# serviceberry3/weiner_slamit_v2

Measured on AMD Instinct MI355X. Metric: frames/sec ORB extract+match @640x480x8lvl, higher is better.
Workload: dtype u8; 1 GPU; BASELINE configs[1]: 640x480 8-level ORB extract (1000 features, FAST 20/7) + brute-force 256-bit Hamming best/second match vs the stream's previous frame; 256 independent streams per GPU per step; distinct_frame_pairs_per_gpu=16, parallelism=streams sharded over 1 GPU(s), no data-path collective

## Files before the change

weiner_slamit_v2_amd/csrc/orb_api.hip:

```cpp
#include <hip/hip_runtime.h>
#include <math.h>
#include <stdio.h>
#include <stdlib.h>
#include <string.h>

#include <algorithm>
#include <vector>

#include "../../include/slamit.h"
#include "orb_plan.h"
#include "slamit_internal.h"

hipError_t orbk_upload_pattern(hipStream_t st);
void orbk_resize(hipStream_t st, const uint8_t* src, int sw, int sh, size_t sstride, size_t sframe,
                 uint8_t* dst, int dw, int dh, size_t dstride, size_t dframe, const int* xofs,
                 const short* ialpha, const int* yofs, const short* ibeta, int nframes);
void orbk_resize_rows4(hipStream_t st, const uint8_t* src, size_t sstride, size_t sframe, int sh, uint8_t* dst, int dw, int dh,
                       size_t dstride, size_t dframe, const uint32_t* d_col, const uint32_t* d_row, int nframes);
void orbk_resize_rows8(hipStream_t st, const uint8_t* src, size_t sstride, size_t sframe, int sh, uint8_t* dst, int dw, int dh,
                       size_t dstride, size_t dframe, const uint32_t* d_col8, const uint32_t* d_row, int nframes);
hipError_t orbk_pyramid_prepare(int smem_bytes);
void orbk_pyramid(hipStream_t st, const OrbLevel* levels, int nlevels, const PyrBox* boxes, const PyrTabs* tabs,
                  int nregions, const uint8_t* img0, size_t img0_stride, size_t img0_frame, uint8_t* pyr, int bufA_bytes,
                  int smem_bytes, int nframes, int l_first, int l_last);
hipError_t orbk_fast_prepare(int max_wcell, int max_hcell);
void orbk_fast(hipStream_t st, const FastTab& tab, int nlevels, const uint32_t* d_cells, int cells_per_frame, const uint8_t* img0,
               size_t img0_stride, size_t img0_frame, const uint8_t* pyr, unsigned long long* cand,
               size_t cand_frame_stride, int* cand_count, int iniTh, int minTh, int max_wcell, int max_hcell, int nframes);
hipError_t orbk_octree_prepare(int node_cap, int key_cap);
void orbk_octree(hipStream_t st, const OrbLevel* levels, int nlevels, const unsigned long long* cand,
                 size_t cand_frame_stride, int* cand_count, uint32_t* ws_xy, uint16_t* ws_node,
                 OrbLevelKp* lkp, size_t kp_frame_stride, int* kp_count, int node_cap, int key_cap, int nframes,
                 int level_override);
void orbk_ic_angle(hipStream_t st, const OrbLevel* levels, int nlevels, const uint8_t* img0, size_t img0_stride,
                   size_t img0_frame, const uint8_t* pyr, OrbLevelKp* lkp, size_t kp_frame_stride,
                   const int* kp_count, int max_kp, int nframes);
void orbk_blur_stream(hipStream_t st, const OrbLevel* levels, const uint32_t* d_tiles, int ntiles, const uint8_t* img0,
                      size_t img0_stride, size_t img0_frame, const uint8_t* pyr, uint8_t* blur, int nframes, bool edge);
void orbk_blur(hipStream_t st, const OrbLevel* levels, const uint32_t* d_tiles, int total_tiles, const uint8_t* img0,
               size_t img0_stride, size_t img0_frame, const uint8_t* pyr, uint8_t* blur, int nframes);
void orbk_describe(hipStream_t st, const OrbLevel* levels, int nlevels, const uint8_t* blur,
                   const OrbLevelKp* lkp, size_t kp_frame_stride, const int* kp_count, slamit_kp* out_kps,
                   uint8_t* out_desc, int out_cap, int* out_n, int max_kp, int nframes);
void orbk_pad(hipStream_t st, const uint8_t* src, int w, int h, size_t sstride, uint8_t* dst);
void orbk_decode_candidates(hipStream_t st, const OrbLevel* levels, int level, const unsigned long long* K, int n,
                            unsigned long long* order_out, int* xys);

namespace {

inline size_t round_up(size_t v, size_t a) { return (v + a - 1) / a * a; }

}

#define ORB_BLUR_SPLIT 1

struct slamit_orb {
    slamit_orb_params p;
    int device;
    hipStream_t stream;
    hipStream_t stream_b;
    hipEvent_t ev_pyr, ev_mid, ev_blur;
    SlamitSwitches sw;
    int nlevels;
    OrbPlan pl;
    bool blur_stream_on;
    uint8_t* d_tables;
    const OrbLevel* d_levels;
    uint8_t* d_pyr;
    uint8_t* d_blur;
    unsigned long long* d_cand;
    uint32_t* d_ws_xy;
    uint16_t* d_ws_node;
    int* d_counts;
// ... 43 lines not shown
        p->ini_th_fast < 1 || p->ini_th_fast > 255 || p->min_th_fast < 1 || p->min_th_fast > 255 ||
        p->width < 0 || p->height < 0 || p->max_batch < 1)
        return slamit_fail(SLAMIT_ERR_ARG, "slamit_orb_create: parameter out of range");
    SLAMIT_USE_DEVICE(device);
    slamit_orb* h = new slamit_orb();
    h->p = *p;
    h->device = device;
    h->sw = slamit_read_switches();
    const int nl = h->nlevels = p->nlevels;
    const char* why = "";
    if (!orb_plan(*p, OrbPlanOptions{h->sw.resize_no8}, h->pl, &why)) {
        delete h;
        return slamit_fail(SLAMIT_ERR_ARG, why);
    }
    const OrbPlan& P = h->pl;
    const bool empty = P.levels.empty();
    h->blur_stream_on = !empty && !h->sw.blur_no_stream;

    const size_t B = (size_t)p->max_batch;
    const size_t counts_bytes = sizeof(int) * ((ORB_CC_PAD + 1) * B * nl + 2 * ORB_CC_PAD);
    h->d_in_stride = round_up((size_t)std::max(p->width, 1), 64);
    h->d_in_frame = h->d_in_stride * std::max(p->height, 1);
    h->scratch_bytes = std::max<size_t>((size_t)(p->width + 38) * (p->height + 38),
                                        (sizeof(unsigned long long) + 3 * sizeof(int)) * (P.cand_frame_stride + 64));
    hipError_t e = hipSuccess;
#define ALLOC(ptr, bytes) if (e == hipSuccess) e = hipMalloc((void**)&(ptr), std::max<size_t>((bytes), 256))
    ALLOC(h->d_tables, P.table_bytes);
    ALLOC(h->d_pyr, P.pyr_frame_total * B);
    ALLOC(h->d_blur, P.blur_frame_total * B + 256);
    ALLOC(h->d_cand, sizeof(unsigned long long) * P.cand_frame_stride * B);
    ALLOC(h->d_ws_xy, sizeof(uint32_t) * P.cand_frame_stride * B);
    ALLOC(h->d_ws_node, sizeof(uint16_t) * P.cand_frame_stride * B);
    ALLOC(h->d_counts, counts_bytes);
    ALLOC(h->d_lkp, sizeof(OrbLevelKp) * P.kp_frame_stride * B);
    ALLOC(h->d_in, h->d_in_frame * B);
    ALLOC(h->d_out_kps, sizeof(slamit_kp) * (size_t)P.max_out * B);
    ALLOC(h->d_out_desc, (size_t)SLAMIT_DESC_BYTES * P.max_out * B);
    ALLOC(h->d_out_n, sizeof(int) * B);
    ALLOC(h->d_scratch, h->scratch_bytes);
#undef ALLOC
    if (e == hipSuccess) e = hipHostMalloc((void**)&h->h_out, 256 + (size_t)B * 256 + (sizeof(slamit_kp) + SLAMIT_DESC_BYTES) * (size_t)P.max_out * B, hipHostMallocDefault);
    if (e == hipSuccess) e = hipStreamCreateWithFlags(&h->stream, hipStreamNonBlocking);
    if (e == hipSuccess) e = hipStreamCreateWithFlags(&h->stream_b, hipStreamNonBlocking);
    if (e == hipSuccess) e = hipEventCreateWithFlags(&h->ev_pyr, hipEventDisableTiming);
    if (e == hipSuccess) e = hipEventCreateWithFlags(&h->ev_mid, hipEventDisableTiming);
    if (e == hipSuccess) e = hipEventCreateWithFlags(&h->ev_blur, hipEventDisableTiming);
    if (e == hipSuccess && P.table_bytes) {
        std::vector<uint8_t> img;
        orb_plan_image(P, h->d_tables, img);
        e = hipMemcpy(h->d_tables, img.data(), img.size(), hipMemcpyHostToDevice);
    }
    h->d_levels = dtab<OrbLevel>(h, P.levels_off);
    if (e == hipSuccess && P.pyr_regions) e = orbk_pyramid_prepare(P.pyr_smem);
    if (e == hipSuccess) e = orbk_upload_pattern(h->stream);
    if (e == hipSuccess) e = orbk_octree_prepare(P.node_cap, P.oct_key_cap);
    if (e == hipSuccess && !empty) e = orbk_fast_prepare(P.max_wcell, P.max_hcell);
    if (e == hipSuccess) e = hipMemset(h->d_counts, 0, counts_bytes);
    if (e == hipSuccess) e = hipStreamSynchronize(h->stream);
    if (e != hipSuccess) {
        orb_free(h);
        return slamit_fail_hip(e, "slamit_orb_create");
    }
    *out = h;
    return SLAMIT_OK;
}
void slamit_orb_destroy(slamit_orb* h) { orb_free(h); }

int slamit_orb_tables(const slamit_orb* h, float* scale, float* inv_scale, float* sigma2, float* inv_sigma2,
                      int32_t* features_per_level) {
    if (!h) return slamit_fail(SLAMIT_ERR_ARG, "slamit_orb_tables: null handle");
    for (int i = 0; i < h->nlevels; ++i) {
        if (scale) scale[i] = h->pl.scale[i];
        if (inv_scale) inv_scale[i] = h->pl.inv_scale[i];
        if (sigma2) sigma2[i] = h->pl.sigma2[i];
        if (inv_sigma2) inv_sigma2[i] = h->pl.inv_sigma2[i];
        if (features_per_level) features_per_level[i] = h->pl.per_level[i];
    }
    return SLAMIT_OK;
}

int slamit_orb_max_keypoints(const slamit_orb* h) { return h ? h->pl.max_out : 0; }

enum { ST_RESIZE = 0, ST_FAST, ST_OCTREE, ST_ANGLE, ST_BLUR, ST_DESCRIBE, ST_COUNT };

static void prof_mark(slamit_orb* h, hipStream_t st, int stage, bool begin) {
    if (!h->prof_on || h->prof_ev.size() >= 2 * 16384) return;
    if (h->prof_on >= 2 && (stage != ST_FAST || h->prof_call % (h->prof_on - 1) != 0)) return;
    hipEvent_t e;
    if (hipEventCreate(&e) != hipSuccess) return;
    hipEventRecord(e, st);
    h->prof_ev.push_back(e);
    if (begin) h->prof_stage.push_back(stage);
}

int slamit_orb_extract_batch_dev(slamit_orb* h, const uint8_t* d_gray, size_t stride, size_t frame_stride,
                                 int nframes, slamit_kp* d_kps, uint8_t* d_desc, int cap, int32_t* d_n_out,
                                 void* stream) {
    if (!h || !d_n_out || nframes < 0) return slamit_fail(SLAMIT_ERR_ARG, "slamit_orb_extract_batch_dev: bad argument");
    if (nframes > h->p.max_batch) return slamit_fail(SLAMIT_ERR_CAPACITY, "slamit_orb_extract_batch_dev: nframes > max_batch");
    if (nframes == 0) return SLAMIT_OK;
    SLAMIT_USE_DEVICE(h->device);
    hipStream_t st = stream ? (hipStream_t)stream : h->stream;
    const int nl = h->nlevels;
    const OrbPlan& P = h->pl;
    if (h->p.width == 0 || h->p.height == 0) {
        HIP_TRY(hipMemsetAsync(d_n_out, 0, sizeof(int) * nframes, st));
        h->last_nframes = 0;
        return SLAMIT_OK;
    }
    if (!d_gray || !d_kps || !d_desc) return slamit_fail(SLAMIT_ERR_ARG, "slamit_orb_extract_batch_dev: null buffer");
    if (cap < P.max_out) return slamit_fail(SLAMIT_ERR_CAPACITY, "slamit_orb_extract_batch_dev: cap < slamit_orb_max_keypoints()");
    if (stride < (size_t)h->p.width || (nframes > 1 && frame_stride < stride * (size_t)h->p.height))
        return slamit_fail(SLAMIT_ERR_ARG, "slamit_orb_extract_batch_dev: stride smaller than the frame");
    if (stride >= ((size_t)1 << 24)) return slamit_fail(SLAMIT_ERR_ARG, "slamit_orb_extract_batch_dev: row pitch of 16 MiB or more");
    int* cand_count = h->d_counts;
    int* kp_count = h->d_counts + (size_t)h->p.max_batch * nl * ORB_CC_PAD;
    if (!h->counters_clean) HIP_TRY(hipMemsetAsync(h->d_counts, 0, sizeof(int) * (size_t)h->p.max_batch * nl * ORB_CC_PAD, st));
    h->counters_clean = false;
    const bool blur_src_aligned = ((((uintptr_t)d_gray) | stride | frame_stride) & 3) == 0;
    auto launch_blur = [&](hipStream_t bs, int l0, int l1) {
        auto strips = [&](const OrbStrips& S) { return dtab<uint32_t>(h, S.off) + 4 * (size_t)S.base[l0]; };
        auto nstrips = [&](const OrbStrips& S) { return S.base[l1] - S.base[l0]; };
        if (h->blur_stream_on && blur_src_aligned) {
            orbk_blur_stream(bs, h->d_levels, strips(P.blur_str), nstrips(P.blur_str), d_gray, stride, frame_stride, h->d_pyr, h->d_blur, nframes, false);
            orbk_blur_stream(bs, h->d_levels, strips(P.blur_edge), nstrips(P.blur_edge), d_gray, stride, frame_stride, h->d_pyr, h->d_blur, nframes, true);
        } else {
            orbk_blur(bs, h->d_levels, strips(P.blur_all), nstrips(P.blur_all), d_gray, stride, frame_stride, h->d_pyr, h->d_blur, nframes);
        }
    };
    prof_mark(h, st, ST_RESIZE, true);
    const bool src0_aligned = ((((uintptr_t)d_gray) | stride | frame_stride) & 3) == 0;
    const bool side = h->prof_on != 1;
    const bool early_blur = side && ORB_BLUR_SPLIT < nl - 1;
    bool early_done = false;
    if (P.rows4_ok && src0_aligned) {
        for (int l = 1; l < nl; ++l) {
            const OrbLevel& S = P.levels[l - 1];
            const OrbLevel& D = P.levels[l];
            const uint8_t* src = l == 1 ? d_gray : h->d_pyr + S.plane_off;
            const OrbResizeTabs& T = P.rs[l];
            if (!T.col8.empty())
                orbk_resize_rows8(st, src, l == 1 ? stride : (size_t)S.stride, l == 1 ? frame_stride : P.pyr_frame_total, S.h,
                                  h->d_pyr + D.plane_off, D.w, D.h, (size_t)D.stride, P.pyr_frame_total, dtab<uint32_t>(h, T.col8_off),
                                  dtab<uint32_t>(h, T.row4_off), nframes);
            else
                orbk_resize_rows4(st, src, l == 1 ? stride : (size_t)S.stride, l == 1 ? frame_stride : P.pyr_frame_total, S.h,
                                  h->d_pyr + D.plane_off, D.w, D.h, (size_t)D.stride, P.pyr_frame_total, dtab<uint32_t>(h, T.col4_off),
                                  dtab<uint32_t>(h, T.row4_off), nframes);
            if (early_blur && l == ORB_BLUR_SPLIT) {
                HIP_TRY(hipEventRecord(h->ev_mid, st));
                HIP_TRY(hipStreamWaitEvent(h->stream_b, h->ev_mid, 0));
                launch_blur(h->stream_b, 0, l + 1);
                early_done = true;
            }
        }
    } else if (P.pyr_regions) {
        orbk_pyramid(st, h->d_levels, nl, dtab<PyrBox>(h, P.boxes_off), dtab<PyrTabs>(h, P.tabs_off), P.pyr_regions, d_gray, stride, frame_stride,
                     h->d_pyr, P.pyr_bufA, P.pyr_smem, nframes, 0, nl - 1);
    } else {
        for (int l = 1; l < nl; ++l) {
            const OrbLevel& S = P.levels[l - 1];
            const OrbLevel& D = P.levels[l];
            const uint8_t* src = l == 1 ? d_gray : h->d_pyr + S.plane_off;
            size_t sstride = l == 1 ? stride : (size_t)S.stride;
            size_t sframe = l == 1 ? frame_stride : P.pyr_frame_total;
            const OrbResizeTabs& T = P.rs[l];
            orbk_resize(st, src, S.w, S.h, sstride, sframe, h->d_pyr + D.plane_off, D.w, D.h, (size_t)D.stride,
                        P.pyr_frame_total, dtab<int>(h, T.xofs_off), dtab<short>(h, T.ialpha_off), dtab<int>(h, T.yofs_off),
                        dtab<short>(h, T.ibeta_off), nframes);
        }
    }
    prof_mark(h, st, ST_RESIZE, false);
    prof_mark(h, st, ST_FAST, true);
    orbk_fast(st, P.fast, nl, dtab<uint32_t>(h, P.cells_off), (int)(P.cells.size() / 4), d_gray, stride, frame_stride, h->d_pyr, h->d_cand,
              P.cand_frame_stride, cand_count, h->p.ini_th_fast, h->p.min_th_fast, P.max_wcell, P.max_hcell, nframes);
    prof_mark(h, st, ST_FAST, false);
    if (side) {
        HIP_TRY(hipEventRecord(h->ev_pyr, st));
        HIP_TRY(hipStreamWaitEvent(h->stream_b, h->ev_pyr, 0));
        launch_blur(h->stream_b, early_done ? ORB_BLUR_SPLIT + 1 : 0, nl);
        HIP_TRY(hipEventRecord(h->ev_blur, h->stream_b));
    }
    prof_mark(h, st, ST_OCTREE, true);
    orbk_octree(st, h->d_levels, nl, h->d_cand, P.cand_frame_stride, cand_count, h->d_ws_xy, h->d_ws_node, h->d_lkp,
                P.kp_frame_stride, kp_count, P.node_cap, P.oct_key_cap, nframes, -1);
    prof_mark(h, st, ST_OCTREE, false);
    prof_mark(h, st, ST_ANGLE, true);
    orbk_ic_angle(st, h->d_levels, nl, d_gray, stride, frame_stride, h->d_pyr, h->d_lkp, P.kp_frame_stride, kp_count,
                  P.max_kp_level, nframes);
    prof_mark(h, st, ST_ANGLE, false);
    if (side) {
        HIP_TRY(hipStreamWaitEvent(st, h->ev_blur, 0));
    } else {
        prof_mark(h, st, ST_BLUR, true);
        launch_blur(st, 0, nl);
        prof_mark(h, st, ST_BLUR, false);
    }
    prof_mark(h, st, ST_DESCRIBE, true);
    orbk_describe(st, h->d_levels, nl, h->d_blur, h->d_lkp, P.kp_frame_stride, kp_count, d_kps, d_desc, cap, d_n_out,
                  P.max_kp_level, nframes);
    prof_mark(h, st, ST_DESCRIBE, false);
    ++h->prof_call;
    HIP_TRY(hipGetLastError());
    h->counters_clean = true;
    h->last_img0 = d_gray; h->last_stride = stride; h->last_frame = frame_stride; h->last_nframes = nframes;
    return SLAMIT_OK;
}

int slamit_orb_extract_batch(slamit_orb* h, const uint8_t* gray, size_t stride, size_t frame_stride, int nframes,
                             slamit_kp* kps, uint8_t* desc, int cap, int* n_out) {
    if (!h || !n_out || nframes < 0) return slamit_fail(SLAMIT_ERR_ARG, "slamit_orb_extract_batch: bad argument");
    if (nframes > h->p.max_batch) return slamit_fail(SLAMIT_ERR_CAPACITY, "slamit_orb_extract_batch: nframes > max_batch");
    if (nframes == 0) return SLAMIT_OK;
    if (h->p.width == 0 || h->p.height == 0) {
        for (int f = 0; f < nframes; ++f) n_out[f] = 0;
        return SLAMIT_OK;
    }
    if (!gray || !kps || !desc) return slamit_fail(SLAMIT_ERR_ARG, "slamit_orb_extract_batch: null buffer");
    if (cap < h->pl.max_out) return slamit_fail(SLAMIT_ERR_CAPACITY, "slamit_orb_extract_batch: cap < slamit_orb_max_keypoints()");
    SLAMIT_USE_DEVICE(h->device);
    const int W = h->p.width, H = h->p.height;
    for (int f = 0; f < nframes; ++f)
        HIP_TRY(hipMemcpy2DAsync(h->d_in + f * h->d_in_frame, h->d_in_stride, gray + (size_t)f * frame_stride, stride, W, H,
                                 hipMemcpyHostToDevice, h->stream));
    int rc = slamit_orb_extract_batch_dev(h, h->d_in, h->d_in_stride, h->d_in_frame, nframes, h->d_out_kps, h->d_out_desc,
                                          h->pl.max_out, h->d_out_n, h->stream);
    if (rc != SLAMIT_OK) return rc;
    const size_t o_k = ((sizeof(int) * (size_t)nframes + 255) & ~(size_t)255), kb = sizeof(slamit_kp) * (size_t)h->pl.max_out * nframes;
    const size_t o_d = (o_k + kb + 255) & ~(size_t)255, db = (size_t)SLAMIT_DESC_BYTES * h->pl.max_out * nframes;
    HIP_TRY(hipMemcpyAsync(h->h_out, h->d_out_n, sizeof(int) * nframes, hipMemcpyDeviceToHost, h->stream));
    HIP_TRY(hipMemcpyAsync(h->h_out + o_k, h->d_out_kps, kb, hipMemcpyDeviceToHost, h->stream));
    HIP_TRY(hipMemcpyAsync(h->h_out + o_d, h->d_out_desc, db, hipMemcpyDeviceToHost, h->stream));
    HIP_TRY(hipStreamSynchronize(h->stream));
// ... 99 lines not shown
```

weiner_slamit_v2_amd/csrc/orb_kernels.hip:

```cpp
#include <hip/hip_runtime.h>
#include <stdint.h>

#include <algorithm>

#include "orb_types.h"
#include "slamit_math.h"
#include "../../include/slamit.h"
#include "../../include/slamit_orb_pattern.h"

#define WAVE 64

__global__ __launch_bounds__(256) void resize_level_kernel(
    const uint8_t* __restrict__ src, int sw, int sh, size_t sstride, size_t sframe,
    uint8_t* __restrict__ dst, int dw, int dh, size_t dstride, size_t dframe,
    const int* __restrict__ xofs, const short* __restrict__ ialpha,
    const int* __restrict__ yofs, const short* __restrict__ ibeta) {
    const int x4 = (blockIdx.x * 64 + (threadIdx.x & 63)) * 4;
    const int y = blockIdx.y * 4 + (threadIdx.x >> 6);
    const int f = blockIdx.z;
    if (x4 >= dw || y >= dh) return;
    const uint8_t* S = src + (size_t)f * sframe;
    int sy = yofs[y];
    int sy0 = min(max(sy, 0), sh - 1), sy1 = min(max(sy + 1, 0), sh - 1);
    const uint8_t* S0 = S + (size_t)sy0 * sstride;
// ... 120 lines not shown
        const unsigned srow = (r & 1) ? (rt[r >> 1].x >> 16) : (rt[r >> 1].x & 0xFFFFu);
        const unsigned ro = __umul24(srow, ss) + b;
        const rs_u4 v = __builtin_amdgcn_raw_buffer_load_b128(rsrc, (int)ro, 0, 0);
        w[r][0] = v.x; w[r][1] = v.y; w[r][2] = v.z; w[r][3] = v.w;
    }
#pragma unroll
    for (int k = 0; k < 2 * RP; ++k) {
        uint32_t h[2][8];
#pragma unroll
        for (int r = 0; r < 2; ++r) {
            const uint32_t* ww = w[2 * k + r];
            const uint32_t a0 = __builtin_amdgcn_alignbyte(ww[1], ww[0], sh), a1 = __builtin_amdgcn_alignbyte(ww[2], ww[1], sh), a2 = __builtin_amdgcn_alignbyte(ww[3], ww[2], sh);
#pragma unroll
            for (int j = 0; j < 4; ++j) h[r][j] = rs_dot2(__builtin_amdgcn_perm(a1, a0, sel[j]), al[j]) >> 4;
#pragma unroll
            for (int j = 4; j < 8; ++j) h[r][j] = rs_dot2(__builtin_amdgcn_perm(a2, a1, sel[j]), al[j]) >> 4;
        }
        const unsigned b0 = rt[k].y & 0xFFFFu, b1 = rt[k].y >> 16;
        uint32_t out[2] = {0, 0};
#pragma unroll
        for (int j = 0; j < 8; ++j) {
            const uint32_t v = ((__umul24(b0, h[0][j]) >> 16) + (__umul24(b1, h[1][j]) >> 16) + 2u) >> 2;
            out[j >> 2] |= (v & 0xFFu) << (8 * (j & 3));
        }
        *reinterpret_cast<uint2*>(D + (__umul24((unsigned)yrow[k], dstride) + 8u * (unsigned)g)) = make_uint2(out[0], out[1]);
    }
}

template <int RP>
__global__ __launch_bounds__(256) void resize_rows8_kernel(
    const uint8_t* __restrict__ src, size_t sstride, size_t sframe,
    uint8_t* __restrict__ dst, size_t dstride, size_t dframe,
    const uint4* __restrict__ coltab, const uint2* __restrict__ rowtab, int ngroups, unsigned inv_groups, int nitems, int dh, unsigned sbytes) {
    const int item = blockIdx.x * 256 + threadIdx.x;
    if (item >= nitems) return;
    rs_item8<RP>(item, src + (size_t)blockIdx.y * sframe, (unsigned)sstride, sbytes, dst + (size_t)blockIdx.y * dframe, (unsigned)dstride, coltab, rowtab,
                 ngroups, inv_groups, dh);
}

void orbk_resize_rows8(hipStream_t st, const uint8_t* src, size_t sstride, size_t sframe, int sh, uint8_t* dst, int dw, int dh,
                       size_t dstride, size_t dframe, const uint32_t* d_col8, const uint32_t* d_row, int nframes) {
    const int ng = (dw + 7) / 8, nitems = ng * ((dh + 2 * RS_RP - 1) / (2 * RS_RP));
    const unsigned inv = (unsigned)((0x100000000ull + (unsigned)ng - 1) / (unsigned)ng);
    hipLaunchKernelGGL(resize_rows8_kernel<RS_RP>, dim3((nitems + 255) / 256, nframes), dim3(256), 0, st, src, sstride, sframe, dst, dstride, dframe,
                       reinterpret_cast<const uint4*>(d_col8), reinterpret_cast<const uint2*>(d_row), ng, inv, nitems, dh, (unsigned)(sstride * (size_t)sh));
}

void orbk_resize_rows4(hipStream_t st, const uint8_t* src, size_t sstride, size_t sframe, int sh, uint8_t* dst, int dw, int dh,
                       size_t dstride, size_t dframe, const uint32_t* d_col, const uint32_t* d_row, int nframes) {
    const int ng = (dw + 3) / 4, nitems = ng * ((dh + 2 * RS_RP - 1) / (2 * RS_RP));
    const unsigned inv = (unsigned)((0x100000000ull + (unsigned)ng - 1) / (unsigned)ng);
    hipLaunchKernelGGL(resize_rows4_kernel<RS_RP>, dim3((nitems + 255) / 256, nframes), dim3(256), 0, st, src, sstride, sframe, dst, dstride, dframe,
                       reinterpret_cast<const uint4*>(d_col), reinterpret_cast<const uint2*>(d_row), ng, inv, nitems, dh, (unsigned)(sstride * (size_t)sh));
}

#define PYR_THREADS 512

__global__ __launch_bounds__(PYR_THREADS) void pyramid_fused_kernel(
    const OrbLevel* __restrict__ levels, int nlevels, const PyrBox* __restrict__ boxes,
    const PyrTabs* __restrict__ tabs, const uint8_t* __restrict__ img0, size_t img0_stride, size_t img0_frame,
    uint8_t* __restrict__ pyr, int bufA_bytes, int l_first, int l_last) {
    extern __shared__ __attribute__((aligned(16))) uint8_t pbuf[];
    uint8_t* buf[2] = {pbuf, pbuf + bufA_bytes};
    const int tx = threadIdx.x & 63, ty = threadIdx.x >> 6;
    const int PYR_ROWS = blockDim.x >> 6, NT = blockDim.x;
    const int frame = blockIdx.y;
    const PyrBox* B = boxes + (size_t)blockIdx.x * nlevels;
    {
        const PyrBox b = B[l_first];
        const int nw = b.nx1 - b.nx0, pitch = (nw + 3) & ~3;
        const uint8_t* S;
        size_t sstride;
        if (l_first == 0) { S = img0 + (size_t)frame * img0_frame; sstride = img0_stride; }
        else { S = pyr + levels[l_first].plane_off + (size_t)frame * levels[l_first].plane_bytes; sstride = (size_t)levels[l_first].stride; }
        const bool aligned = ((((uintptr_t)S) | sstride) & 3) == 0;
        const int w0 = levels[l_first].w;
        if (aligned) {
            const int nd = pitch >> 2;
            for (int y = b.ny0 + ty; y < b.ny1; y += PYR_ROWS)
                for (int d = tx; d < nd; d += 64) {
                    const int x = b.nx0 + 4 * d;
                    uint32_t v;
                    if (x + 4 <= w0) v = *reinterpret_cast<const uint32_t*>(S + (size_t)y * sstride + x);
                    else { v = 0; for (int j = 0; j < 4; ++j) if (x + j < w0) v |= (uint32_t)S[(size_t)y * sstride + x + j] << (8 * j); }
                    *reinterpret_cast<uint32_t*>(&buf[0][(y - b.ny0) * pitch + 4 * d]) = v;
                }
        } else {
            for (int y = b.ny0 + ty; y < b.ny1; y += PYR_ROWS)
                for (int x = b.nx0 + tx; x < b.nx1; x += 64)
                    buf[0][(y - b.ny0) * pitch + (x - b.nx0)] = S[(size_t)y * sstride + x];
        }
    }
    __syncthreads();
    for (int l = l_first + 1; l <= l_last; ++l) {
        const PyrBox b = B[l], pb = B[l - 1];
        const OrbLevel& L = levels[l];
        const int sw = levels[l - 1].w, sh = levels[l - 1].h;
        const PyrTabs T = tabs[l];
        const uint8_t* src = buf[(l - 1 - l_first) & 1];
        uint8_t* dst = buf[(l - l_first) & 1];
        const int spitch = ((pb.nx1 - pb.nx0) + 3) & ~3, dpitch = ((b.nx1 - b.nx0) + 3) & ~3;
        uint8_t* plane = pyr + L.plane_off + (size_t)frame * L.plane_bytes;
        const int nw = b.nx1 - b.nx0;
        int cx0[4], cx1[4], ca0[4], ca1[4];
        unsigned ownmask = 0;
#pragma unroll
// ... 1481 lines not shown
```

weiner_slamit_v2_amd/csrc/orb_plan.cc:

```cpp
#include "orb_plan.h"

#include <math.h>
#include <string.h>

#include <algorithm>

namespace {

inline int cv_round(double v) { return (int)lrint(v); }
inline size_t round_up(size_t v, size_t a) { return (v + a - 1) / a * a; }

inline short sat_short(float v) {
    int iv = cv_round((double)v);
    return (short)(iv < -32768 ? -32768 : iv > 32767 ? 32767 : iv);
}

void plan_scales(const slamit_orb_params& p, OrbPlan& P) {
    const int nl = p.nlevels;
    const double scaleFactor = (double)p.scale_factor;
    P.scale.assign(nl, 1.f); P.sigma2.assign(nl, 1.f); P.inv_scale.assign(nl, 1.f); P.inv_sigma2.assign(nl, 1.f);
    for (int i = 1; i < nl; ++i) {
        P.scale[i] = (float)(P.scale[i - 1] * scaleFactor);
        P.sigma2[i] = P.scale[i] * P.scale[i];
    }
// ... 205 lines not shown
            P.rows4_ok = false;
            T.col4.clear(); T.row4.clear();
        }
        if (o.resize_no8 || !rows8_table(D.w, S.w, (size_t)D.stride, T.xofs.data(), T.ialpha.data(), T.col8)) T.col8.clear();
    }
}

void plan_pyramid_boxes(const slamit_orb_params& p, OrbPlan& P) {
    const int nl = (int)P.levels.size(), last = nl - 1;
    if (nl < 2) return;
    const int GX = std::max(1, (p.width + 127) / 128), GY = std::max(1, (p.height + 95) / 96);
    std::vector<PyrBox> boxes((size_t)GX * GY * nl);
    bool ok = true;
    size_t capA = 16, capB = 16;
    for (int gy = 0; gy < GY && ok; ++gy)
        for (int gx = 0; gx < GX && ok; ++gx) {
            PyrBox* B = &boxes[((size_t)gy * GX + gx) * nl];
            for (int l = 0; l <= last; ++l) {
                const OrbLevel& L = P.levels[l];
                B[l].ox0 = (int16_t)((long)gx * L.w / GX); B[l].ox1 = (int16_t)((long)(gx + 1) * L.w / GX);
                B[l].oy0 = (int16_t)((long)gy * L.h / GY); B[l].oy1 = (int16_t)((long)(gy + 1) * L.h / GY);
                if (l == 0) { B[l].ox0 = B[l].ox1 = B[l].oy0 = B[l].oy1 = 0; }
                else if (B[l].ox1 <= B[l].ox0 || B[l].oy1 <= B[l].oy0) ok = false;
            }
            B[last].nx0 = B[last].ox0; B[last].nx1 = B[last].ox1;
            B[last].ny0 = B[last].oy0; B[last].ny1 = B[last].oy1;
            for (int l = last; l > 0 && ok; --l) {
                const std::vector<int32_t> &XO = P.rs[l].xofs, &YO = P.rs[l].yofs;
                const int sw = P.levels[l - 1].w, sh = P.levels[l - 1].h;
                int sx0 = XO[B[l].nx0], sx1 = std::min(XO[B[l].nx1 - 1] + 1, sw - 1) + 1;
                int sy0 = std::min(std::max(YO[B[l].ny0], 0), sh - 1);
                int sy1 = std::min(std::max(YO[B[l].ny1 - 1] + 1, 0), sh - 1) + 1;
                if (l - 1 > 0) {
                    sx0 = std::min(sx0, (int)B[l - 1].ox0); sx1 = std::max(sx1, (int)B[l - 1].ox1);
                    sy0 = std::min(sy0, (int)B[l - 1].oy0); sy1 = std::max(sy1, (int)B[l - 1].oy1);
                }
                if (l - 1 == 0) sx0 &= ~3;
                B[l - 1].nx0 = (int16_t)sx0; B[l - 1].nx1 = (int16_t)sx1; B[l - 1].ny0 = (int16_t)sy0; B[l - 1].ny1 = (int16_t)sy1;
            }
            for (int l = 0; l <= last; ++l) {
                if (l > 0 && (B[l].nx1 - B[l].nx0 > 256 || B[l].ny1 - B[l].ny0 > 256)) ok = false;
                size_t bytes = (size_t)(((B[l].nx1 - B[l].nx0) + 3) & ~3) * (B[l].ny1 - B[l].ny0);
                if (l & 1) capB = std::max(capB, bytes); else capA = std::max(capA, bytes);
            }
        }
    const int bufA = (int)round_up(capA, 16), smem = bufA + (int)round_up(capB, 16);
    if (!ok || smem > 150 * 1024) return;
    P.pyr_regions = GX * GY;
    P.pyr_bufA = bufA;
    P.pyr_smem = smem;
    P.boxes.swap(boxes);
}

void plan_table_block(OrbPlan& P) {
    size_t off = 0;
    auto take = [&](size_t bytes) { const size_t at = round_up(off, 256); off = at + bytes; return at; };
    const int nl = (int)P.levels.size();
    P.levels_off = take(sizeof(OrbLevel) * nl);
    P.cells_off = take(sizeof(uint32_t) * P.cells.size());
    for (OrbStrips* S : {&P.blur_all, &P.blur_str, &P.blur_edge}) S->off = take(sizeof(uint32_t) * S->tab.size());
    for (int l = 1; l < nl; ++l) {
        OrbResizeTabs& T = P.rs[l];
        T.xofs_off = take(sizeof(int32_t) * T.xofs.size()); T.ialpha_off = take(sizeof(int16_t) * T.ialpha.size());
        T.yofs_off = take(sizeof(int32_t) * T.yofs.size()); T.ibeta_off = take(sizeof(int16_t) * T.ibeta.size());
        T.col4_off = take(sizeof(uint32_t) * T.col4.size()); T.row4_off = take(sizeof(uint32_t) * T.row4.size());
        T.col8_off = take(sizeof(uint32_t) * T.col8.size());
    }
    P.boxes_off = take(sizeof(PyrBox) * P.boxes.size());
    P.tabs_off = take(P.pyr_regions ? sizeof(PyrTabs) * nl : 0);
    P.table_bytes = round_up(off, 256);
}

}

bool orb_plan(const slamit_orb_params& p, const OrbPlanOptions& o, OrbPlan& plan, const char** why) {
    plan = OrbPlan();
    OrbPlan& P = plan;
    P.node_cap = 8; P.max_kp_level = 1;
    P.rows4_ok = true;
    plan_scales(p, P);
    P.max_out = p.nfeatures + 3 * p.nlevels;
    const bool empty = p.width == 0 || p.height == 0;
    if (!empty && !plan_levels(p, P, why)) return false;
    P.oct_key_cap = octree_key_cap(P.node_cap, p.width, p.height);
    if (orbk_octree_smem(P.node_cap, P.oct_key_cap) > 160 * 1024 - 1024 || P.node_cap >= 4096) {
        *why = "slamit_orb_create: nfeatures too large for the LDS octree";
        return false;
    }
    fast_cells(P);
    blur_strips(P);
    plan_resize(o, P);
    plan_pyramid_boxes(p, P);
    plan_table_block(P);
    return true;
}

void orb_plan_image(const OrbPlan& P, const uint8_t* base, std::vector<uint8_t>& img) {
    img.assign(P.table_bytes, 0);
    auto put = [&](size_t off, const void* src, size_t bytes) { if (bytes) memcpy(img.data() + off, src, bytes); };
    auto put_vec = [&](size_t off, const auto& v) { put(off, v.data(), sizeof(v[0]) * v.size()); };
    put(P.levels_off, P.levels.data(), sizeof(OrbLevel) * P.levels.size());
    put_vec(P.cells_off, P.cells);
    for (const OrbStrips* S : {&P.blur_all, &P.blur_str, &P.blur_edge}) put_vec(S->off, S->tab);
    for (size_t l = 1; l < P.rs.size(); ++l) {
        const OrbResizeTabs& T = P.rs[l];
        put_vec(T.xofs_off, T.xofs); put_vec(T.ialpha_off, T.ialpha); put_vec(T.yofs_off, T.yofs); put_vec(T.ibeta_off, T.ibeta);
        put_vec(T.col4_off, T.col4); put_vec(T.row4_off, T.row4); put_vec(T.col8_off, T.col8);
    }
    put_vec(P.boxes_off, P.boxes);
    if (!P.pyr_regions) return;
    std::vector<PyrTabs> tabs(P.levels.size(), PyrTabs{nullptr, nullptr, nullptr, nullptr});
    auto at = [&](size_t off) { return (uintptr_t)base + off; };
    for (size_t l = 1; l < tabs.size(); ++l) {
        const OrbResizeTabs& T = P.rs[l];
        tabs[l].xofs = reinterpret_cast<const int32_t*>(at(T.xofs_off)); tabs[l].ialpha = reinterpret_cast<const int16_t*>(at(T.ialpha_off));
        tabs[l].yofs = reinterpret_cast<const int32_t*>(at(T.yofs_off)); tabs[l].ibeta = reinterpret_cast<const int16_t*>(at(T.ibeta_off));
    }
    put_vec(P.tabs_off, tabs);
}
```

weiner_slamit_v2_amd/csrc/orb_plan.h:

```cpp
#ifndef SLAMIT_ORB_PLAN_H
#define SLAMIT_ORB_PLAN_H

#include <stddef.h>
#include <stdint.h>

#include <vector>

#include "../../include/slamit.h"
#include "orb_types.h"

struct OrbPlanOptions {
    bool resize_no8;
};

struct OrbStrips {
    std::vector<uint32_t> tab;
    int base[ORB_MAX_LEVELS + 1];
    size_t off;
};

struct OrbResizeTabs {
    std::vector<int32_t> xofs, yofs;
    std::vector<int16_t> ialpha, ibeta;
    std::vector<uint32_t> col4, row4;
    std::vector<uint32_t> col8;
    size_t xofs_off, ialpha_off, yofs_off, ibeta_off, col4_off, row4_off, col8_off;
};

struct OrbPlan {
    std::vector<float> scale, inv_scale, sigma2, inv_sigma2;
    std::vector<int> per_level;
    std::vector<OrbLevel> levels;
    size_t pyr_frame_total, blur_frame_total, cand_frame_stride, kp_frame_stride;
    int max_out, node_cap, oct_key_cap, max_kp_level, max_wcell, max_hcell;
    std::vector<uint32_t> cells;
    size_t cells_off;
    FastTab fast;
    OrbStrips blur_all, blur_str, blur_edge;
    std::vector<OrbResizeTabs> rs;
    bool rows4_ok;
    int pyr_regions, pyr_bufA, pyr_smem;
    std::vector<PyrBox> boxes;
    size_t levels_off, boxes_off, tabs_off;
    size_t table_bytes;
};

bool orb_plan(const slamit_orb_params& p, const OrbPlanOptions& o, OrbPlan& plan, const char** why);

void orb_plan_image(const OrbPlan& plan, const uint8_t* base, std::vector<uint8_t>& img);

#endif
```

weiner_slamit_v2_amd/csrc/orb_types.h:

```cpp
#ifndef SLAMIT_ORB_TYPES_H
#define SLAMIT_ORB_TYPES_H

#include <stddef.h>
#include <stdint.h>

#ifdef __HIPCC__
#define ORB_HD __host__ __device__
#else
#define ORB_HD
#endif

#define ORB_MAX_LEVELS 16
#define ORB_MAX_ROOTS 8
#define ORB_MIN_BORDER 16
#define ORB_CELL_MAX 59
#define ORB_TILE_MAX (ORB_CELL_MAX + 6)
#define ORB_CC_PAD 32
#define BLUR_STEPS 4
#define ORB_BLUR_STRIP_H (16 * BLUR_STEPS)

ORB_HD inline size_t orbk_octree_node_bytes(int node_cap) {
    return ((size_t)node_cap * (8 + 2 * 8 + 2 * 4 + 4 * 4 + 5 * 4 + 4 + 4) + 64 + 15) & ~(size_t)15;
}
ORB_HD inline size_t orbk_octree_smem(int node_cap, int key_cap) { return orbk_octree_node_bytes(node_cap) + (size_t)key_cap * 6; }
#define OCT_LDS_KEYS_MAX 10240
#define OCT_LDS_KEYS_MIN 2048
#define OCT_LDS_BUDGET (78 * 1024)

struct OrbLevel {
    int32_t w, h;
    int32_t stride;
    int32_t quota;
    uint64_t plane_off;
    uint64_t plane_bytes;
    uint64_t blur_off;
    uint64_t blur_bytes;
    int32_t nCols, nRows, wCell, hCell;
    int32_t maxBorderX, maxBorderY;
    int32_t cell_base;
    int32_t ncells;
    int32_t blur_tile_base;
    uint64_t cand_off;
    int32_t cand_cap;
    int32_t nIni;
    float hX;
    int32_t rootUL[ORB_MAX_ROOTS], rootUR[ORB_MAX_ROOTS];
    int32_t boxH;
    int32_t kp_off, kp_cap;
    float scale;
    float patch_size;
};

struct FastLevel {
    int32_t cell_base, nCols, wCell, hCell, maxBorderX, maxBorderY, stride, cand_cap;
    uint64_t plane_off, plane_bytes, cand_off;
};
struct FastTab { FastLevel lv[ORB_MAX_LEVELS]; };

struct PyrBox {
    int16_t ox0, oy0, ox1, oy1;
    int16_t nx0, ny0, nx1, ny1;
};
struct PyrTabs {
    const int32_t* xofs; const int16_t* ialpha;
    const int32_t* yofs; const int16_t* ibeta;
};

struct OrbLevelKp {
    int16_t x, y;
    float response;
    float angle;
    float cs, sn;
};

#endif
```

Before: 310,600 frames/s.

## Fuse pyramid resize levels into banded multi-level kernel with LDS intermediates

Replaces the per-level resize launches with a banded kernel that computes several consecutive pyramid levels in one launch. Each block owns a horizontal band and keeps intermediate level rows in double-buffered LDS tiles, including halo rows, so the next level is read from LDS instead of global memory. The plan splits the levels into two segments, and the early blur fork now happens after the first segment. This cuts kernel launches and global round-trips between levels, at the cost of recomputing halo rows across bands and extra LDS pressure.

```diff
diff --git a/weiner_slamit_v2_amd/csrc/orb_api.hip b/weiner_slamit_v2_amd/csrc/orb_api.hip
--- a/weiner_slamit_v2_amd/csrc/orb_api.hip
+++ b/weiner_slamit_v2_amd/csrc/orb_api.hip
@@ -19,6 +19,9 @@
                        size_t dstride, size_t dframe, const uint32_t* d_col, const uint32_t* d_row, int nframes);
 void orbk_resize_rows8(hipStream_t st, const uint8_t* src, size_t sstride, size_t sframe, int sh, uint8_t* dst, int dw, int dh,
                        size_t dstride, size_t dframe, const uint32_t* d_col8, const uint32_t* d_row, int nframes);
+hipError_t orbk_pyramid_bands_prepare(int smem_bytes);
+void orbk_pyramid_bands(hipStream_t st, const BandTab& tab, const uint8_t* d_tables, const BandRows* d_rows, int first, int last, int nbands,
+                        const uint8_t* src, size_t sstride, size_t sframe, int sh, uint8_t* pyr, size_t pyr_frame, int tile0, int smem, int nframes);
 hipError_t orbk_pyramid_prepare(int smem_bytes);
 void orbk_pyramid(hipStream_t st, const OrbLevel* levels, int nlevels, const PyrBox* boxes, const PyrTabs* tabs,
                   int nregions, const uint8_t* img0, size_t img0_stride, size_t img0_frame, uint8_t* pyr, int bufA_bytes,
@@ -168,6 +171,7 @@
     }
     h->d_levels = dtab<OrbLevel>(h, P.levels_off);
     if (e == hipSuccess && P.pyr_regions) e = orbk_pyramid_prepare(P.pyr_smem);
+    for (const OrbBandSeg& G : P.bands) if (e == hipSuccess) e = orbk_pyramid_bands_prepare(G.smem);
     if (e == hipSuccess) e = orbk_upload_pattern(h->stream);
     if (e == hipSuccess) e = orbk_octree_prepare(P.node_cap, P.oct_key_cap);
     if (e == hipSuccess && !empty) e = orbk_fast_prepare(P.max_wcell, P.max_hcell);
@@ -248,8 +252,24 @@
     const bool src0_aligned = ((((uintptr_t)d_gray) | stride | frame_stride) & 3) == 0;
     const bool side = h->prof_on != 1;
     const bool early_blur = side && ORB_BLUR_SPLIT < nl - 1;
-    bool early_done = false;
-    if (P.rows4_ok && src0_aligned) {
+    int early_done = -1;
+    auto fork_early_blur = [&](int l) -> hipError_t {
+        hipError_t e = hipEventRecord(h->ev_mid, st);
+        if (e == hipSuccess) e = hipStreamWaitEvent(h->stream_b, h->ev_mid, 0);
+        if (e != hipSuccess) return e;
+        launch_blur(h->stream_b, 0, l + 1);
+        early_done = l;
+        return hipSuccess;
+    };
+    if (!P.bands.empty() && src0_aligned) {
+        for (const OrbBandSeg& G : P.bands) {
+            const OrbLevel& S = P.levels[G.first];
+            orbk_pyramid_bands(st, P.band_tab, h->d_tables, dtab<BandRows>(h, G.rows_off), G.first, G.last, G.nbands,
+                               G.first == 0 ? d_gray : h->d_pyr + S.plane_off, G.first == 0 ? stride : (size_t)S.stride,
+                               G.first == 0 ? frame_stride : P.pyr_frame_total, S.h, h->d_pyr, P.pyr_frame_total, G.tile0, G.smem, nframes);
+            if (early_blur && G.last < nl - 1 && early_done < 0) HIP_TRY(fork_early_blur(G.last));
+        }
+    } else if (P.rows4_ok && src0_aligned) {
         for (int l = 1; l < nl; ++l) {
             const OrbLevel& S = P.levels[l - 1];
             const OrbLevel& D = P.levels[l];
@@ -263,12 +283,7 @@
                 orbk_resize_rows4(st, src, l == 1 ? stride : (size_t)S.stride, l == 1 ? frame_stride : P.pyr_frame_total, S.h,
                                   h->d_pyr + D.plane_off, D.w, D.h, (size_t)D.stride, P.pyr_frame_total, dtab<uint32_t>(h, T.col4_off),
                                   dtab<uint32_t>(h, T.row4_off), nframes);
-            if (early_blur && l == ORB_BLUR_SPLIT) {
-                HIP_TRY(hipEventRecord(h->ev_mid, st));
-                HIP_TRY(hipStreamWaitEvent(h->stream_b, h->ev_mid, 0));
-                launch_blur(h->stream_b, 0, l + 1);
-                early_done = true;
-            }
+            if (early_blur && l == ORB_BLUR_SPLIT) HIP_TRY(fork_early_blur(l));
         }
     } else if (P.pyr_regions) {
         orbk_pyramid(st, h->d_levels, nl, dtab<PyrBox>(h, P.boxes_off), dtab<PyrTabs>(h, P.tabs_off), P.pyr_regions, d_gray, stride, frame_stride,
@@ -294,7 +309,7 @@
     if (side) {
         HIP_TRY(hipEventRecord(h->ev_pyr, st));
         HIP_TRY(hipStreamWaitEvent(h->stream_b, h->ev_pyr, 0));
-        launch_blur(h->stream_b, early_done ? ORB_BLUR_SPLIT + 1 : 0, nl);
+        launch_blur(h->stream_b, early_done + 1, nl);
         HIP_TRY(hipEventRecord(h->ev_blur, h->stream_b));
     }
     prof_mark(h, st, ST_OCTREE, true);
diff --git a/weiner_slamit_v2_amd/csrc/orb_kernels.hip b/weiner_slamit_v2_amd/csrc/orb_kernels.hip
--- a/weiner_slamit_v2_amd/csrc/orb_kernels.hip
+++ b/weiner_slamit_v2_amd/csrc/orb_kernels.hip
@@ -196,6 +196,120 @@
     const unsigned inv = (unsigned)((0x100000000ull + (unsigned)ng - 1) / (unsigned)ng);
     hipLaunchKernelGGL(resize_rows4_kernel<RS_RP>, dim3((nitems + 255) / 256, nframes), dim3(256), 0, st, src, sstride, sframe, dst, dstride, dframe,
                        reinterpret_cast<const uint4*>(d_col), reinterpret_cast<const uint2*>(d_row), ng, inv, nitems, dh, (unsigned)(sstride * (size_t)sh));
+}
+
+#define BAND_THREADS 256
+
+template <bool FROM_LDS, bool TO_LDS>
+__device__ __forceinline__ void band_item(const int item, const BandLevel& V, const uint8_t* __restrict__ tables, const BandRows R,
+                                          const __amdgpu_buffer_rsrc_t rsrc, const unsigned ss, const uint8_t* stile, const int srow0,
+                                          const unsigned spitch, uint8_t* dtile, uint8_t* D) {
+    const int yq = (int)__umulhi((unsigned)item, V.inv_groups);
+    const int g = item - yq * V.ngroups;
+    const uint8_t* ct = tables + V.col_off + 80u * (unsigned)g;
+    const uint4 c0 = *reinterpret_cast<const uint4*>(ct), c1 = *reinterpret_cast<const uint4*>(ct + 16u), c2 = *reinterpret_cast<const uint4*>(ct + 32u),
+                c3 = *reinterpret_cast<const uint4*>(ct + 48u);
+    const uint32_t c4x = *reinterpret_cast<const uint32_t*>(ct + 64u);
+    int yrow[4];
+    uint2 rt[4];
+    const uint8_t* rtab = tables + V.row_off;
+#pragma unroll
+    for (int r = 0; r < 4; ++r) {
+        yrow[r] = min((int)R.cmp0 + 4 * yq + r, (int)R.cmp1 - 1);
+        rt[r] = *reinterpret_cast<const uint2*>(rtab + 8u * (unsigned)yrow[r]);
+    }
+    const unsigned b = c0.x & 0xFFFFu, sh = (c0.x >> 16) & 3u;
+    const uint32_t sel[8] = {c0.y, c0.z, c0.w, c1.x, c1.y, c1.z, c1.w, c2.x}, al[8] = {c2.y, c2.z, c2.w, c3.x, c3.y, c3.z, c3.w, c4x};
+    uint32_t w[8][4];
+#pragma unroll
+    for (int r = 0; r < 8; ++r) {
+        const unsigned srow = (r & 1) ? (rt[r >> 1].x >> 16) : (rt[r >> 1].x & 0xFFFFu);
+        if (FROM_LDS) {
+            const uint32_t* p = reinterpret_cast<const uint32_t*>(stile + (__umul24(srow - (unsigned)srow0, spitch) + b));
+            w[r][0] = p[0]; w[r][1] = p[1]; w[r][2] = p[2]; w[r][3] = p[3];
+        } else {
+            const rs_u4 v = __builtin_amdgcn_raw_buffer_load_b128(rsrc, (int)(__umul24(srow, ss) + b), 0, 0);
+            w[r][0] = v.x; w[r][1] = v.y; w[r][2] = v.z; w[r][3] = v.w;
+        }
+    }
+#pragma unroll
+    for (int k = 0; k < 4; ++k) {
+        uint32_t h[2][8];
+#pragma unroll
+        for (int r = 0; r < 2; ++r) {
+            const uint32_t* ww = w[2 * k + r];
+            const uint32_t a0 = __builtin_amdgcn_alignbyte(ww[1], ww[0], sh), a1 = __builtin_amdgcn_alignbyte(ww[2], ww[1], sh), a2 = __builtin_amdgcn_alignbyte(ww[3], ww[2], sh);
+#pragma unroll
+            for (int j = 0; j < 4; ++j) h[r][j] = rs_dot2(__builtin_amdgcn_perm(a1, a0, sel[j]), al[j]) >> 4;
+#pragma unroll
+            for (int j = 4; j < 8; ++j) h[r][j] = rs_dot2(__builtin_amdgcn_perm(a2, a1, sel[j]), al[j]) >> 4;
+        }
+        const unsigned b0 = rt[k].y & 0xFFFFu, b1 = rt[k].y >> 16;
+        uint32_t out[2] = {0, 0};
+#pragma unroll
+        for (int j = 0; j < 8; ++j) {
+            const uint32_t v = ((__umul24(b0, h[0][j]) >> 16) + (__umul24(b1, h[1][j]) >> 16) + 2u) >> 2;
+            out[j >> 2] |= (v & 0xFFu) << (8 * (j & 3));
+        }
+        if (TO_LDS) *reinterpret_cast<uint2*>(dtile + (__umul24((unsigned)(yrow[k] - (int)R.cmp0), (unsigned)V.pitch) + 8u * (unsigned)g)) = make_uint2(out[0], out[1]);
+        if (yrow[k] >= (int)R.own0 && yrow[k] < (int)R.own1)
+            *reinterpret_cast<uint2*>(D + (__umul24((unsigned)yrow[k], (unsigned)V.dstride) + 8u * (unsigned)g)) = make_uint2(out[0], out[1]);
+    }
+}
+
+__global__ __launch_bounds__(BAND_THREADS) void pyramid_bands_kernel(
+    const BandTab tab, const uint8_t* __restrict__ tables, const BandRows* __restrict__ rows, const int first, const int last, const int nbands,
+    const uint8_t* __restrict__ src, const unsigned sstride, const size_t sframe, const unsigned sbytes,
+    uint8_t* __restrict__ pyr, const size_t pyr_frame, const int tile0, const int xcd_frames) {
+    extern __shared__ __attribute__((aligned(16))) uint8_t band_lds[];
+    int frame, band;
+    if (xcd_frames) {
+        const unsigned w = blockIdx.x, k = w >> 3, fq = k / (unsigned)nbands;
+        frame = (int)(8u * fq + ((w + fq) & 7u));
+        if (frame >= xcd_frames) return;
+        band = (int)(k - fq * (unsigned)nbands);
+    } else { band = blockIdx.x; frame = blockIdx.y; }
+    const int nlv = last - first;
+    const BandRows* BR = rows + (size_t)band * nlv;
+    const __amdgpu_buffer_rsrc_t rsrc = __builtin_amdgcn_make_buffer_rsrc(const_cast<uint8_t*>(src + (size_t)frame * sframe), 0, sbytes, 0x00020000);
+    uint8_t* planes = pyr + (size_t)frame * pyr_frame;
+    int srow0 = 0;
+    for (int k = 0; k < nlv; ++k) {
+        const BandLevel& V = tab.lv[first + 1 + k];
+        const BandRows R = BR[k];
+        uint8_t* dtile = band_lds + ((k & 1) ? tile0 : 0);
+        const uint8_t* stile = band_lds + ((k & 1) ? 0 : tile0);
+        const unsigned spitch = (unsigned)tab.lv[first + k].pitch;
+        uint8_t* D = planes + V.plane_off;
+        const int nitems = V.ngroups * (((int)R.cmp1 - (int)R.cmp0 + 3) >> 2);
+        const bool to_lds = k + 1 < nlv;
+        for (int item = threadIdx.x; item < nitems; item += BAND_THREADS) {
+            if (k == 0) {
+                if (to_lds) band_item<false, true>(item, V, tables, R, rsrc, sstride, stile, srow0, spitch, dtile, D);
+                else band_item<false, false>(item, V, tables, R, rsrc, sstride, stile, srow0, spitch, dtile, D);
+            } else {
+                if (to_lds) band_item<true, true>(item, V, tables, R, rsrc, sstride, stile, srow0, spitch, dtile, D);
+                else band_item<true, false>(item, V, tables, R, rsrc, sstride, stile, srow0, spitch, dtile, D);
+            }
+        }
+        srow0 = R.cmp0;
+        if (to_lds) __syncthreads();
+    }
+}
+
+void orbk_pyramid_bands(hipStream_t st, const BandTab& tab, const uint8_t* d_tables, const BandRows* d_rows, int first, int last, int nbands,
+                        const uint8_t* src, size_t sstride, size_t sframe, int sh, uint8_t* pyr, size_t pyr_frame, int tile0, int smem, int nframes) {
+    const int xcd_frames = nframes >= 16 ? nframes : 0;
+    const dim3 grid = xcd_frames ? dim3((unsigned)(((nframes + 7) / 8) * 8) * (unsigned)nbands) : dim3(nbands, nframes);
+    hipLaunchKernelGGL(pyramid_bands_kernel, grid, dim3(BAND_THREADS), smem, st, tab, d_tables, d_rows, first, last, nbands, src, (unsigned)sstride, sframe,
+                       (unsigned)(sstride * (size_t)sh), pyr, pyr_frame, tile0, xcd_frames);
+}
+
+hipError_t orbk_pyramid_bands_prepare(int smem_bytes) {
+    static int prepared = 0;
+    if (smem_bytes <= prepared) return hipSuccess;
+    prepared = smem_bytes;
+    return hipFuncSetAttribute(reinterpret_cast<const void*>(pyramid_bands_kernel), hipFuncAttributeMaxDynamicSharedMemorySize, smem_bytes);
 }
 
 #define PYR_THREADS 512
diff --git a/weiner_slamit_v2_amd/csrc/orb_plan.cc b/weiner_slamit_v2_amd/csrc/orb_plan.cc
--- a/weiner_slamit_v2_amd/csrc/orb_plan.cc
+++ b/weiner_slamit_v2_amd/csrc/orb_plan.cc
@@ -281,6 +281,37 @@
     P.boxes.swap(boxes);
 }
 
+#ifndef ORB_BAND_COUNT
+#define ORB_BAND_COUNT 8
+#define ORB_BAND_SPLIT 2
+#endif
+
+inline int band_pitch(int w) { return (int)round_up((size_t)((w + 7) / 8) * 8, 16); }
+
+void plan_bands(OrbPlan& P) {
+    const int nl = (int)P.levels.size();
+    if (nl < 2 || !P.rows4_ok) return;
+    for (int l = 1; l < nl; ++l) {
+        const OrbResizeTabs& T = P.rs[l];
+        if (T.col8.empty() || T.row4.empty() || P.levels[l].h >= 65536) return;
+        BandLevel& V = P.band_tab.lv[l];
+        V.ngroups = (P.levels[l].w + 7) / 8;
+        V.inv_groups = (uint32_t)((0x100000000ull + (unsigned)V.ngroups - 1) / (unsigned)V.ngroups);
+        V.dstride = P.levels[l].stride;
+        V.pitch = band_pitch(P.levels[l].w);
+        V.plane_off = P.levels[l].plane_off;
+    }
+    const int split = ORB_BAND_SPLIT > 0 && ORB_BAND_SPLIT < nl - 1 ? ORB_BAND_SPLIT : nl - 1;
+    std::vector<OrbBandSeg> segs;
+    for (int first = 0; first < nl - 1; first = segs.back().last) {
+        segs.emplace_back();
+        int nb = ORB_BAND_COUNT;
+        while (!orb_plan_band_segment(P, first, first == 0 ? split : nl - 1, nb, ORB_BAND_LDS_BUDGET, segs.back()))
+            if ((nb *= 2) > 8 * ORB_BAND_COUNT) return;
+    }
+    P.bands.swap(segs);
+}
+
 void plan_table_block(OrbPlan& P) {
     size_t off = 0;
     auto take = [&](size_t bytes) { const size_t at = round_up(off, 256); off = at + bytes; return at; };
@@ -297,6 +328,9 @@
     }
     P.boxes_off = take(sizeof(PyrBox) * P.boxes.size());
     P.tabs_off = take(P.pyr_regions ? sizeof(PyrTabs) * nl : 0);
+    for (OrbBandSeg& G : P.bands) G.rows_off = take(sizeof(BandRows) * G.rows.size());
+    if (!P.bands.empty())
+        for (int l = 1; l < nl; ++l) { P.band_tab.lv[l].col_off = P.rs[l].col8_off; P.band_tab.lv[l].row_off = P.rs[l].row4_off; }
     P.table_bytes = round_up(off, 256);
 }
 
@@ -320,8 +354,41 @@
     blur_strips(P);
     plan_resize(o, P);
     plan_pyramid_boxes(p, P);
+    plan_bands(P);
     plan_table_block(P);
     return true;
+}
+
+bool orb_plan_band_segment(const OrbPlan& P, int first, int last, int nbands, size_t lds_budget, OrbBandSeg& seg) {
+    const int nl = (int)P.levels.size(), nlv = last - first;
+    if (first < 0 || last >= nl || nlv < 1 || nbands < 1) return false;
+    seg = OrbBandSeg();
+    seg.first = first; seg.last = last; seg.nbands = nbands;
+    seg.rows.assign((size_t)nbands * nlv, BandRows());
+    size_t tile[2] = {0, 0};
+    for (int b = 0; b < nbands; ++b) {
+        BandRows* R = &seg.rows[(size_t)b * nlv];
+        int need0 = 0, need1 = 0;
+        for (int l = last; l > first; --l) {
+            const int h = P.levels[l].h;
+            if (h < nbands || h >= 65536 || P.rs[l].row4.size() < 2 * (size_t)h) return false;
+            const int own0 = (int)((long)b * h / nbands), own1 = (int)((long)(b + 1) * h / nbands);
+            const int cmp0 = l == last ? own0 : std::min(own0, need0), cmp1 = l == last ? own1 : std::max(own1, need1);
+            R[l - first - 1] = BandRows{(uint16_t)own0, (uint16_t)own1, (uint16_t)cmp0, (uint16_t)cmp1};
+            need0 = 65535; need1 = 0;
+            for (int y = cmp0; y < cmp1; ++y) {
+                const uint32_t s = P.rs[l].row4[2 * (size_t)y];
+                need0 = std::min(need0, (int)(s & 0xFFFFu)); need1 = std::max(need1, (int)(s >> 16) + 1);
+            }
+            if (l < last) {
+                size_t& t = tile[(l - first - 1) & 1];
+                t = std::max(t, (size_t)(cmp1 - cmp0) * band_pitch(P.levels[l].w) + ORB_BAND_SLACK);
+            }
+        }
+    }
+    seg.tile0 = (int)round_up(tile[0], 16);
+    seg.smem = seg.tile0 + (int)round_up(tile[1], 16);
+    return (size_t)seg.smem <= lds_budget;
 }
 
 void orb_plan_image(const OrbPlan& P, const uint8_t* base, std::vector<uint8_t>& img) {
@@ -337,6 +404,7 @@
         put_vec(T.col4_off, T.col4); put_vec(T.row4_off, T.row4); put_vec(T.col8_off, T.col8);
     }
     put_vec(P.boxes_off, P.boxes);
+    for (const OrbBandSeg& G : P.bands) put_vec(G.rows_off, G.rows);
     if (!P.pyr_regions) return;
     std::vector<PyrTabs> tabs(P.levels.size(), PyrTabs{nullptr, nullptr, nullptr, nullptr});
     auto at = [&](size_t off) { return (uintptr_t)base + off; };
diff --git a/weiner_slamit_v2_amd/csrc/orb_plan.h b/weiner_slamit_v2_amd/csrc/orb_plan.h
--- a/weiner_slamit_v2_amd/csrc/orb_plan.h
+++ b/weiner_slamit_v2_amd/csrc/orb_plan.h
@@ -27,6 +27,13 @@
     size_t xofs_off, ialpha_off, yofs_off, ibeta_off, col4_off, row4_off, col8_off;
 };
 
+struct OrbBandSeg {
+    int first, last, nbands;
+    std::vector<BandRows> rows;
+    int tile0, smem;
+    size_t rows_off;
+};
+
 struct OrbPlan {
     std::vector<float> scale, inv_scale, sigma2, inv_sigma2;
     std::vector<int> per_level;
@@ -42,11 +49,15 @@
     int pyr_regions, pyr_bufA, pyr_smem;
     std::vector<PyrBox> boxes;
     size_t levels_off, boxes_off, tabs_off;
+    std::vector<OrbBandSeg> bands;
+    BandTab band_tab;
     size_t table_bytes;
 };
 
 bool orb_plan(const slamit_orb_params& p, const OrbPlanOptions& o, OrbPlan& plan, const char** why);
 
+bool orb_plan_band_segment(const OrbPlan& plan, int first, int last, int nbands, size_t lds_budget, OrbBandSeg& seg);
+
 void orb_plan_image(const OrbPlan& plan, const uint8_t* base, std::vector<uint8_t>& img);
 
 #endif
diff --git a/weiner_slamit_v2_amd/csrc/orb_types.h b/weiner_slamit_v2_amd/csrc/orb_types.h
--- a/weiner_slamit_v2_amd/csrc/orb_types.h
+++ b/weiner_slamit_v2_amd/csrc/orb_types.h
@@ -66,6 +66,17 @@
     const int32_t* yofs; const int16_t* ibeta;
 };
 
+struct BandLevel {
+    uint64_t col_off, row_off;
+    uint64_t plane_off;
+    int32_t ngroups, dstride, pitch;
+    uint32_t inv_groups;
+};
+struct BandTab { BandLevel lv[ORB_MAX_LEVELS]; };
+struct BandRows { uint16_t own0, own1, cmp0, cmp1; };
+#define ORB_BAND_LDS_BUDGET (78 * 1024)
+#define ORB_BAND_SLACK 16
+
 struct OrbLevelKp {
     int16_t x, y;
     float response;
```

After: 316,500 frames/s, median of 6. +1.9%, better.
